# pixray/pixray

Measured on AMD Instinct MI355X. Metric: optimisation iters/sec, VQGAN 256^2 + ViT-B/32 + 64 cutouts, higher is better.
Workload: dtype fp16

## Files before the change

include/prx.h:

```cpp
#ifndef PRX_H_
#define PRX_H_
#include <stddef.h>
#include <stdint.h>

#ifdef __cplusplus
extern "C" {
#endif

#define PRX_ABI_VERSION 3

typedef void* prx_stream_t;

const char* prx_last_error(void);
int prx_abi_version(void);
int prx_device_info(int* cu_count, char* arch_name, int arch_name_len);


#define PRX_ACT_NONE 0
#define PRX_ACT_QUICKGELU 1
#define PRX_ACT_MUL_DQUICKGELU 2
#define PRX_ACT_RELU 3
#define PRX_ACT_MUL_RELUMASK 4
#define PRX_ACT_RELUMASK_POST 5
#define PRX_ACT_GELU 6
// ... 54 lines not shown
                           void* dST, int lddst, int rows, int cols, prx_stream_t s);
int prx_k_upsample2x_bwd(const float* hi, float* low, int NB, int Hl, int Wl, int C, prx_stream_t s);
int prx_k_nchw_to_nhwc(const float* in, float* out_f32, void* out_bf16, int NB, int C, int HW, int Cpad,
                       prx_stream_t s);
int prx_k_nhwc_to_nchw(const float* in, int ldc, float* out, int NB, int C, int HW, prx_stream_t s);
int prx_k_image_head_fwd(const float* x, int ldc, float* img, int NB, int C, int HW, prx_stream_t s);
int prx_k_image_head_bwd(const float* x, int ldc, const float* gimg, float* dx, void* dx_bf16, int ldo, int NB, int C,
                         int HW, prx_stream_t s);
int prx_k_mha_fwd(const void* qkv, void* out, int N, int T, int C, int heads, prx_stream_t s);
int prx_k_mha_bwd(const void* qkv, const void* dout, void* dqkv, int N, int T, int C, int heads, prx_stream_t s);

int prx_k_groupnorm_fwd_op(const void* x, const float* gamma, const float* beta, double* stats, void* out16, float* out_f32,
                           int NB, int P, int C, int swish, float eps, int zero_stats, int stats_ready, int h16, int s16,
                           prx_stream_t s);
int prx_k_groupnorm_bwd_op(const void* g, const void* x, const float* gamma, const float* beta, const double* fstats,
                           double* bstats, const void* add, float* dx, void* dx16, int NB, int P, int C, int swish, float eps,
                           int zero_stats, int stats_ready, int h16, int s16, prx_stream_t s);
int prx_k_layernorm_fwd_op(const void* x, long long ldx, const float* gamma, const float* beta, void* out16, float* out_f32,
                           float* mean, float* rstd, int rows, int C, float eps, int h16, int s16, prx_stream_t s);
int prx_k_layernorm_bwd_op(const void* g, long long ldg, const void* x, long long ldx, const float* gamma, const float* mean,
                           const float* rstd, const void* add, long long ldadd, float* dx, long long lddx, void* dx16,
                           long long lddxb, int rows, int C, int h16, int add_every, int s16, prx_stream_t s);
int prx_k_mha_fwd_op(const void* qkv, void* out, int N, int T, int C, int heads, int h16, prx_stream_t s);
int prx_k_mha_bwd_op(const void* qkv, const void* dout, void* dqkv, int N, int T, int C, int heads, int h16, prx_stream_t s);
int prx_k_mha_fwd_gen_op(const void* qkv, void* out, float* lse, int N, int T, int C, int heads, int h16, prx_stream_t s);
int prx_k_mha_bwd_gen_op(const void* qkv, const void* out, const void* dout, const float* lse, void* dqkv, int N, int T, int C,
                         int heads, int h16, prx_stream_t s);
int prx_k_mha_fwd_causal_op(const void* qkv, void* out, int N, int T, int C, int heads, int h16, prx_stream_t s);
int prx_k_softmax_rows_op(const float* S, int lds_, float scale, void* P, int ldp, void* PT, int ldpt, int rows, int cols,
                          int prec, prx_stream_t s);
int prx_k_softmax_rows_bwd_op(const void* P, int ldp, const float* dP, int lddp, float scale, void* dS, int ldds, void* dST,
                              int lddst, int rows, int cols, int prec, prx_stream_t s);
int prx_k_transpose_op(const void* in, int ldin, void* out, int ldout, int R, int C, int f32, prx_stream_t s);
int prx_k_upsample2x_bwd_op(const void* hi, float* low, void* low16, int NB, int Hl, int Wl, int C, int h16, int s16,
                            prx_stream_t s);
int prx_k_nchw_to_nhwc_op(const float* in, float* out_f32, void* out16, int NB, int C, int HW, int Cpad, int h16, prx_stream_t s);
int prx_k_image_head_bwd_op(const float* x, int ldc, const float* gimg, float* dx, void* dx16, int ldo, int NB, int C, int HW,
                            int h16, const float* gscale, prx_stream_t s);
int prx_k_image_head_bwd_im2col(const float* x, int ldc, const float* gimg, void* col, int ldk, int C, int H, int W, int h16,
                                const float* gscale, prx_stream_t s);
int prx_k_grad_scale(const float* g, size_t n, float* part, int nparts, int target_log2, float* scale2, prx_stream_t s);
int prx_k_grad_scale_multi(const float* const* gs, const size_t* ns, int count, float* part, int nparts_each, int target_log2,
                           float* scale2, prx_stream_t s);
int prx_k_scale_dev(float* x, size_t n, const float* scale, void* out16, int h16, prx_stream_t s);
int prx_k_f32_to_op16(const float* in, void* out16, size_t n, int h16, prx_stream_t s);
int prx_k_add_f32(const float* a, const float* b, float* out, size_t n, prx_stream_t s);

int prx_k_rn_pack_conv3x3(const float* w, void* Wf, void* Wd, int Cout, int Cin, int prec, prx_stream_t s);
int prx_k_stem1_fwd(const float* cut, const float* mm, const float* w, const float* b, void* out, int N, int S, int CO, int prec,
                    prx_stream_t s);
int prx_k_stem1_bwd(const void* g, const float* w, float* dY, int N, int S, int CO, const float* oscale_dev, int prec, prx_stream_t s);
int prx_k_avgpool2_fwd(const void* x, void* out, int N, int H, int W, int C, int prec, prx_stream_t s);
int prx_k_avgpool2_bwd(const float* g, const void* mask, float* dx_f32, void* dx_op, int N, int H, int W, int C, int prec,
                       prx_stream_t s);
int prx_k_relu_mask(float* g, const void* out, void* g_op, size_t n, int prec, prx_stream_t s);
int prx_k_tokens_fwd(const float* x, const float* pos, void* t, int N, int P, int C, int prec, prx_stream_t s);
int prx_k_tokens_bwd(const float* dt, float* dx, int N, int P, int C, int prec, prx_stream_t s);
int prx_k_tok0_gather(const void* t, void* out, int N, int T, int C, int prec, prx_stream_t s);
int prx_k_tok0_scatter(const void* g0, void* dt, int N, int T, int C, int prec, prx_stream_t s);
int prx_k_minmax(const float* x, size_t n, float* part, int nparts, float* mm, prx_stream_t s);
int prx_k_patchify_fwd(const float* cut, const float* mm, void* A, int prec, int N, int S, int P, int T, float m0, float m1, float m2,
                       float s0, float s1, float s2, prx_stream_t s);
int prx_k_patchify_bwd_reduce(const float* cut, const float* mm, const float* dA, double* acc, int N, int S, int P, int T, float m0,
                              float m1, float m2, float s0, float s1, float s2, prx_stream_t s);
int prx_k_patchify_bwd_apply(const float* cut, const float* mm, const float* dA, const double* acc, float* gcut, int N, int S, int P,
                             int T, float m0, float m1, float m2, float s0, float s1, float s2, prx_stream_t s);
// ... 285 lines not shown
```

pixray_amd/csrc/api_kernels.hip:

```cpp
#include "common.h"
#include "norms.h"
#include "elementwise.h"
#include "attention.h"
#include "resnet.h"
#include "cutouts.h"
#include "vgg.h"
#include "vit.h"
#include "clip_text.h"
#include "prompt_vq.h"
#include "vqgan.h"
#include "vqgan_enc.h"
#include "../../include/prx.h"

#define S_(x) ((hipStream_t)(x))
#define B_(x) ((bf16_t*)(x))
#define CB_(x) ((const bf16_t*)(x))

extern "C" {

int prx_k_groupnorm_fwd(const float* x, const float* gamma, const float* beta, double* stats, void* out_bf16,
                        float* out_f32, int NB, int P, int C, int swish, float eps, prx_stream_t s) {
    return prx_groupnorm_fwd(x, gamma, beta, stats, B_(out_bf16), out_f32, NB, P, C, swish, eps, S_(s));
}
int prx_k_groupnorm_bwd(const float* g, const float* x, const float* gamma, const float* beta, const double* fstats,
                        double* bstats, const float* add, float* dx, int NB, int P, int C, int swish, float eps,
                        prx_stream_t s) {
    return prx_groupnorm_bwd(g, x, gamma, beta, fstats, bstats, add, dx, nullptr, NB, P, C, swish, eps, S_(s));
}
int prx_k_layernorm_fwd(const float* x, long long ldx, const float* gamma, const float* beta, void* out_bf16,
                        float* out_f32, float* mean, float* rstd, int rows, int C, float eps, prx_stream_t s) {
    return prx_layernorm_fwd(x, ldx, gamma, beta, B_(out_bf16), out_f32, mean, rstd, rows, C, eps, S_(s));
}
int prx_k_layernorm_bwd(const float* g, long long ldg, const float* x, long long ldx, const float* gamma,
                        const float* mean, const float* rstd, const float* add, long long ldadd, float* dx,
                        long long lddx, int rows, int C, prx_stream_t s) {
    return prx_layernorm_bwd(g, ldg, x, ldx, gamma, mean, rstd, add, ldadd, dx, lddx, nullptr, 0, rows, C, S_(s));
}
int prx_k_transpose_bf16(const void* in, int ldin, void* out, int ldout, int R, int C, prx_stream_t s) {
    return prx_transpose_op(in, ldin, out, ldout, R, C, PRX_PREC_BF16, S_(s));
}
int prx_k_softmax_rows(const float* S, int lds_, float scale, void* P, int ldp, void* PT, int ldpt, int rows, int cols,
                       prx_stream_t s) {
    return prx_softmax_rows(S, lds_, scale, P, ldp, PT, ldpt, rows, cols, PRX_PREC_BF16, S_(s));
// ... 59 lines not shown
}
int prx_k_layernorm_bwd_op(const void* g, long long ldg, const void* x, long long ldx, const float* gamma, const float* mean,
                           const float* rstd, const void* add, long long ldadd, float* dx, long long lddx, void* dx16,
                           long long lddxb, int rows, int C, int h16, int add_every, int s16, prx_stream_t s) {
    return prx_layernorm_bwd(g, ldg, x, ldx, gamma, mean, rstd, add, ldadd, dx, lddx, B_(dx16), lddxb, rows, C, S_(s), h16,
                             add_every, s16);
}
int prx_k_mha_fwd_op(const void* qkv, void* out, int N, int T, int C, int heads, int h16, prx_stream_t s) {
    return prx_mha_fwd(CB_(qkv), B_(out), N, T, C, heads, S_(s), h16);
}
int prx_k_mha_bwd_op(const void* qkv, const void* dout, void* dqkv, int N, int T, int C, int heads, int h16, prx_stream_t s) {
    return prx_mha_bwd(CB_(qkv), CB_(dout), B_(dqkv), N, T, C, heads, S_(s), h16);
}
int prx_k_mha_fwd_gen_op(const void* qkv, void* out, float* lse, int N, int T, int C, int heads, int h16, prx_stream_t s) {
    return prx_mha_fwd_gen(CB_(qkv), B_(out), lse, N, T, C, heads, S_(s), h16);
}
int prx_k_mha_bwd_gen_op(const void* qkv, const void* out, const void* dout, const float* lse, void* dqkv, int N, int T, int C,
                         int heads, int h16, prx_stream_t s) {
    return prx_mha_bwd_gen(CB_(qkv), CB_(out), CB_(dout), lse, B_(dqkv), N, T, C, heads, S_(s), h16);
}
int prx_k_mha_fwd_causal_op(const void* qkv, void* out, int N, int T, int C, int heads, int h16, prx_stream_t s) {
    return prx_mha_fwd_causal(CB_(qkv), B_(out), N, T, C, heads, S_(s), h16);
}
int prx_k_softmax_rows_op(const float* S, int lds_, float scale, void* P, int ldp, void* PT, int ldpt, int rows, int cols,
                          int prec, prx_stream_t s) {
    PRX_REQUIRE(prec_valid(prec), "softmax_rows: unknown precision %d", prec);
    return prx_softmax_rows(S, lds_, scale, P, ldp, PT, ldpt, rows, cols, prec, S_(s));
}
int prx_k_softmax_rows_bwd_op(const void* P, int ldp, const float* dP, int lddp, float scale, void* dS, int ldds, void* dST,
                              int lddst, int rows, int cols, int prec, prx_stream_t s) {
    PRX_REQUIRE(prec_valid(prec), "softmax_rows_bwd: unknown precision %d", prec);
    return prx_softmax_rows_bwd(P, ldp, dP, lddp, scale, dS, ldds, dST, lddst, rows, cols, prec, S_(s));
}
int prx_k_transpose_op(const void* in, int ldin, void* out, int ldout, int R, int C, int f32, prx_stream_t s) {
    return prx_transpose_op(in, ldin, out, ldout, R, C, f32, S_(s));
}
int prx_k_upsample2x_bwd_op(const void* hi, float* low, void* low16, int NB, int Hl, int Wl, int C, int h16, int s16,
                            prx_stream_t s) {
    return prx_upsample2x_bwd(hi, low, B_(low16), NB, Hl, Wl, C, S_(s), h16, s16);
}
int prx_k_nchw_to_nhwc_op(const float* in, float* out_f32, void* out16, int NB, int C, int HW, int Cpad, int h16, prx_stream_t s) {
    return prx_nchw_to_nhwc(in, out_f32, B_(out16), NB, C, HW, Cpad, S_(s), h16);
}
int prx_k_image_head_bwd_op(const float* x, int ldc, const float* gimg, float* dx, void* dx16, int ldo, int NB, int C, int HW,
                            int h16, const float* gscale, prx_stream_t s) {
    return prx_image_head_bwd(x, ldc, gimg, dx, B_(dx16), ldo, NB, C, HW, S_(s), h16, gscale);
}
int prx_k_image_head_bwd_im2col(const float* x, int ldc, const float* gimg, void* col, int ldk, int C, int H, int W, int h16,
                                const float* gscale, prx_stream_t s) {
    return prx_image_head_bwd_im2col(x, ldc, gimg, B_(col), ldk, C, H, W, S_(s), h16, gscale);
}
int prx_k_grad_scale(const float* g, size_t n, float* part, int nparts, int target_log2, float* scale2, prx_stream_t s) {
    return prx_grad_scale(g, n, part, nparts, target_log2, scale2, S_(s));
}
int prx_k_grad_scale_multi(const float* const* gs, const size_t* ns, int count, float* part, int nparts_each, int target_log2,
                           float* scale2, prx_stream_t s) {
    return prx_grad_scale_multi(gs, ns, count, part, nparts_each, target_log2, scale2, S_(s));
}
int prx_k_scale_dev(float* x, size_t n, const float* scale, void* out16, int h16, prx_stream_t s) {
    return prx_scale_dev(x, n, scale, S_(s), B_(out16), h16);
}
int prx_k_f32_to_op16(const float* in, void* out16, size_t n, int h16, prx_stream_t s) {
    return prx_f32_to_bf16(in, B_(out16), n, S_(s), h16);
}
int prx_k_add_f32(const float* a, const float* b, float* out, size_t n, prx_stream_t s) {
    return prx_add_f32(a, b, out, n, S_(s));
// ... 104 lines not shown
```

pixray_amd/csrc/vqgan.hip:

```cpp
#include "vqgan.h"
#include "gemm.h"
#include "norms.h"
#include "elementwise.h"
#include "prompt_vq.h"
#include "vit.h"
#include <vector>
#include <memory>
#include <stdlib.h>

namespace {

template <typename TOp>
__global__ __launch_bounds__(256) void pack_conv3x3_kernel(const float* __restrict__ w, TOp* __restrict__ Wf,
                                                           TOp* __restrict__ Wd, int Cout, int Cin, int CoP) {
    const size_t total_f = (size_t)Cout * 9 * Cin;
    const size_t total_d = (size_t)Cin * 9 * CoP;
    for (size_t i = (size_t)blockIdx.x * blockDim.x + threadIdx.x; i < total_f + total_d;
         i += (size_t)gridDim.x * blockDim.x) {
        if (i < total_f) {
            int ci = (int)(i % Cin);
            int tap = (int)((i / Cin) % 9);
            int co = (int)(i / ((size_t)9 * Cin));
            Wf[i] = op_cvt<TOp>(w[(((size_t)co * Cin + ci) * 3 + tap / 3) * 3 + tap % 3]);
        } else {
            size_t j = i - total_f;
            int co = (int)(j % CoP);
            int tap = (int)((j / CoP) % 9);
            int ci = (int)(j / ((size_t)9 * CoP));
            int ky = 2 - tap / 3, kx = 2 - tap % 3;
            Wd[j] = op_cvt<TOp>((co < Cout) ? w[(((size_t)co * Cin + ci) * 3 + ky) * 3 + kx] : 0.f);
        }
    }
}

__global__ __launch_bounds__(256) void colminmax_kernel(const float* __restrict__ w, float* __restrict__ mn,
                                                        float* __restrict__ mx, int rows, int D) {
// ... 6 lines not shown

}

int prx_vqgan_pack_conv3x3(const float* w, void* Wf, void* Wd, int Cout, int Cin, int CoP, int prec, hipStream_t s) {
    PRX_REQUIRE(prec_valid(prec), "vqgan pack_conv3x3: unknown precision %d", prec);
    PRX_OP_DISPATCH(prec_is_f32(prec), prec_is_h16(prec), TO,
                    hipLaunchKernelGGL(pack_conv3x3_kernel<TO>, dim3(1024), dim3(256), 0, s, w, (TO*)Wf, (TO*)Wd, Cout, Cin, CoP));
    PRX_LAUNCH_CHECK();
    return 0;
}
int prx_colminmax(const float* w, float* mn, float* mx, int rows, int D, hipStream_t s) {
    hipLaunchKernelGGL(colminmax_kernel, dim3(ceil_div(D, 256)), dim3(256), 0, s, w, mn, mx, rows, D);
    PRX_LAUNCH_CHECK();
    return 0;
}

static inline int pad8(int P) { return (P + 7) & ~7; }

struct Conv3 { int Cin, Cout, CoP; void *Wf, *Wd; float* b; };
struct Conv1 { int Cin, Cout; void *W, *WT; float* b; };
struct GN { int C; float *g, *b; double *stats, *bstats; int id; };

struct ResBlock {
    int Cin, Cout, rh, rw;
    GN n1, n2; Conv3 c1, c2; Conv1 sc; bool has_sc;
    void *x_in, *h1, *scbuf, *out;
    void *x_in_bf, *out_bf;
};
struct AttnBlock {
    int C, rh, rw;
    GN n; Conv1 qkv, proj;
    void* x_in; void *qkvb, *Pm, *PT; void* out; void* out_bf;
    void* qkvT;
};
struct UpBlock { int C, rh, rw; Conv3 c; void *x_in, *out; void *x_in_bf, *out_bf; };

struct Stage { int kind; int idx; };

struct PrxVqgan {
    int zc, D, NC, ch, out_ch, h0, w0, H, W, nstage;
    int prec;
    int f32, h16;
    int lean;
    float* gs;
    GemmCtx gctx;
    std::vector<void*> allocs;
    float *codebook, *cnorm, *zmin, *zmax;
    Conv1 pq; Conv3 conv_in, conv_out; GN norm_out;
    std::vector<ResBlock> res; std::vector<AttnBlock> attn; std::vector<UpBlock> ups; std::vector<Stage> stages;
    float *zq, *y, *dzq; void* h_in; int* idx; void *pqo_bf, *h_in_bf, *dpq_bf;
    float *pmin; int* pidx;
    void* a;
    void *tA, *tB, *tC, *tD, *dqkv, *dy8;
    void *dycol, *Wd_col;
    float* S;
    void *g0, *g1, *g2;
    void *g0b, *g1b, *g2b;
    double* all_stats; int n_gn;
    float* ws; size_t ws_bytes;
    void* x_last;
};

namespace {
template <typename Tp>
int dalloc(PrxVqgan* v, Tp** p, size_t count) {
    void* q = nullptr;
    PRX_CHECK_HIP(hipMalloc(&q, std::max<size_t>(count, 1) * sizeof(Tp)));
    v->allocs.push_back(q);
    *p = (Tp*)q;
    return 0;
}
#define VALLOC(ptr, count) do { int _r = dalloc(v, &(ptr), (count)); if (_r) return _r; } while (0)
int dalloc_op(PrxVqgan* v, void** p, size_t count) {
    void* q = nullptr;
    PRX_CHECK_HIP(hipMalloc(&q, std::max<size_t>(count, 1) * op_esz(v->f32)));
    v->allocs.push_back(q);
// ... 58 lines not shown
    if ((r = make_gn(v, rb.n2, Cout, cur, s))) return r;
    if ((r = make_conv3(v, rb.c2, Cout, Cout, cur, s))) return r;
    const size_t P = (size_t)rh * rw;
    if (rb.has_sc) {
        if ((r = make_conv1(v, rb.sc, Cin, Cout, cur, s))) return r;
        VALLOC_S(rb.scbuf, P * Cout);
    }
    VALLOC_S(rb.h1, P * Cout); VALLOC_S(rb.out, P * Cout);
    v->stages.push_back({0, (int)v->res.size()});
    v->res.push_back(rb);
    return 0;
}
int make_attn(PrxVqgan* v, int C, int rh, int rw, WCursor& cur, hipStream_t s) {
    AttnBlock ab{};
    ab.C = C; ab.rh = rh; ab.rw = rw;
    int r;
    if ((r = make_gn(v, ab.n, C, cur, s))) return r;
    const float *wq, *bq, *wk, *bk, *wv, *bv;
    NEXTW(cur, wq); NEXTW(cur, bq); NEXTW(cur, wk); NEXTW(cur, bk); NEXTW(cur, wv); NEXTW(cur, bv);
    float *wcat, *bcat;
    VALLOC(wcat, (size_t)3 * C * C); VALLOC(bcat, 3 * C);
    const float* ws_[3] = {wq, wk, wv}; const float* bs_[3] = {bq, bk, bv};
    for (int i = 0; i < 3; ++i) {
        PRX_CHECK_HIP(hipMemcpyAsync(wcat + (size_t)i * C * C, ws_[i], sizeof(float) * C * C, hipMemcpyDeviceToDevice, s));
        PRX_CHECK_HIP(hipMemcpyAsync(bcat + i * C, bs_[i], sizeof(float) * C, hipMemcpyDeviceToDevice, s));
    }
    ab.qkv.Cin = C; ab.qkv.Cout = 3 * C; ab.qkv.b = bcat;
    VALLOC_OP(ab.qkv.W, (size_t)3 * C * C); VALLOC_OP(ab.qkv.WT, (size_t)3 * C * C);
    if ((r = prx_pack_op(wcat, ab.qkv.W, (size_t)3 * C * C, v->prec, s))) return r;
    if ((r = prx_pack_transpose_op(wcat, ab.qkv.WT, 3 * C, C, v->prec, s))) return r;
    if ((r = make_conv1(v, ab.proj, C, C, cur, s))) return r;
    const size_t P = (size_t)rh * rw;
    const size_t P8 = (size_t)pad8((int)P);
    VALLOC_OP(ab.qkvb, P * 3 * C); VALLOC_OP(ab.Pm, P * P8); VALLOC_OP(ab.PT, P * P8); VALLOC_S(ab.out, P * C);
    VALLOC_OP(ab.qkvT, (size_t)3 * C * P8);
    PRX_CHECK_HIP(hipMemsetAsync(ab.qkvT, 0, (size_t)3 * C * P8 * op_esz(v->f32), s));
    PRX_CHECK_HIP(hipMemsetAsync(ab.Pm, 0, P * P8 * op_esz(v->f32), s));
    PRX_CHECK_HIP(hipMemsetAsync(ab.PT, 0, P * P8 * op_esz(v->f32), s));
    v->stages.push_back({1, (int)v->attn.size()});
    v->attn.push_back(ab);
    return 0;
}
int make_up(PrxVqgan* v, int C, int rh, int rw, WCursor& cur, hipStream_t s) {
    UpBlock ub{};
    ub.C = C; ub.rh = rh; ub.rw = rw;
    int r;
    if ((r = make_conv3(v, ub.c, C, C, cur, s))) return r;
    VALLOC_S(ub.out, (size_t)rh * rw * C);
    v->stages.push_back({2, (int)v->ups.size()});
    v->ups.push_back(ub);
    return 0;
}
}

int prx_vqgan_create_impl(PrxVqgan** out, int ch, const int* ch_mult, int n_mult, int num_res_blocks, int attn_res,
                          int resolution, int z_channels, int embed_dim, int n_embed, int out_ch, int h0, int w0,
                          int precision, const float* const* w, int n_w, hipStream_t s) {
    PRX_REQUIRE(h0 >= 1 && w0 >= 1, "vqgan_create: bad latent size %dx%d", h0, w0);
    PRX_REQUIRE(prec_valid(precision), "vqgan_create: unknown precision %d", precision);
    PRX_REQUIRE(embed_dim == z_channels, "vqgan_create: embed_dim must equal z_channels");
    PrxVqgan* v = new PrxVqgan();
    std::unique_ptr<PrxVqgan> guard(v);
    v->prec = precision; v->f32 = prec_is_f32(precision); v->h16 = prec_is_h16(precision);
    v->gs = nullptr;
    { const char* e = getenv("PRX_LEAN"); v->lean = (v->h16 && !(e && atoi(e) == 0)) ? 1 : 0; }
    v->n_gn = 0; v->zc = z_channels; v->D = embed_dim; v->NC = n_embed; v->ch = ch; v->out_ch = out_ch; v->h0 = h0; v->w0 = w0;
    WCursor cur{w, n_w, 0};
    int r;
    const float* cb; NEXTW(cur, cb);
    if ((r = copyf(v, &v->codebook, cb, (size_t)n_embed * embed_dim, s))) return r;
    VALLOC(v->cnorm, n_embed); VALLOC(v->zmin, embed_dim); VALLOC(v->zmax, embed_dim);
    if ((r = prx_sqnorm_rows(v->codebook, v->cnorm, n_embed, embed_dim, s))) return r;
    if ((r = prx_colminmax(v->codebook, v->zmin, v->zmax, n_embed, embed_dim, s))) return r;
    if ((r = make_conv1(v, v->pq, embed_dim, z_channels, cur, s))) return r;
    int block_in = ch * ch_mult[n_mult - 1];
    int rh = h0, rw = w0;
    if ((r = make_conv3(v, v->conv_in, z_channels, block_in, cur, s))) return r;
    if ((r = make_res(v, block_in, block_in, rh, rw, cur, s))) return r;
    if ((r = make_attn(v, block_in, rh, rw, cur, s))) return r;
    if ((r = make_res(v, block_in, block_in, rh, rw, cur, s))) return r;
    int nominal = resolution >> (n_mult - 1);
    for (int lvl = n_mult - 1; lvl >= 0; --lvl) {
        int block_out = ch * ch_mult[lvl];
        for (int b = 0; b < num_res_blocks + 1; ++b) {
            if ((r = make_res(v, block_in, block_out, rh, rw, cur, s))) return r;
            block_in = block_out;
            if (nominal == attn_res) { if ((r = make_attn(v, block_in, rh, rw, cur, s))) return r; }
        }
        if (lvl != 0) {
            rh *= 2; rw *= 2; nominal *= 2;
            if ((r = make_up(v, block_in, rh, rw, cur, s))) return r;
        }
    }
    v->H = rh; v->W = rw;
    if ((r = make_gn(v, v->norm_out, block_in, cur, s))) return r;
    if ((r = make_conv3(v, v->conv_out, block_in, out_ch, cur, s))) return r;
    PRX_REQUIRE(cur.pos == n_w, "vqgan_create: %d weight tensors given, %d consumed", n_w, cur.pos);
    const size_t P0 = (size_t)h0 * w0, PH = (size_t)rh * rw;
// ... 168 lines not shown
    bool sr = nx && nx->C == v->conv_in.Cout && fusable(v, nx->C);
    void* x = v->h_in;
    void* x_bf = v->h_in_bf;
    for (int si = 0; si < (int)v->stages.size(); ++si) {
        const Stage& st = v->stages[si];
        nx = first_norm(v, si + 1);
        if (st.kind == 0) {
            ResBlock& b = v->res[st.idx];
            const int P = b.rh * b.rw;
            b.x_in = x; b.x_in_bf = x_bf;
            if ((r = gn_fwd(v, b.n1, x, P, 1, s, sr))) return r;
            if ((r = conv3_fwd(v, b.c1, v->a, false, b.rh, b.rw, false, nullptr, b.h1, b.Cout, s, nullptr, &b.n2))) return r;
            const void* resid = x;
            if (b.has_sc) {
                PRX_REQUIRE(x_bf != nullptr, "vqgan: missing bf16 twin for the shortcut input");
                GemmDesc d; d.A = x_bf; d.lda = b.Cin; d.B = b.sc.W; d.ldb = b.Cin; d.M = P; d.N = b.Cout; d.K = b.Cin;
                d.bias_n = b.sc.b; out_stream(v, d, b.scbuf, b.Cout, nullptr);
                if ((r = vg(v, d, s))) return r;
                resid = b.scbuf;
            }
            if ((r = gn_fwd(v, b.n2, b.h1, P, 1, s, fusable(v, b.Cout)))) return r;
            if ((r = conv3_fwd(v, b.c2, v->a, false, b.rh, b.rw, false, resid, b.out, b.Cout, s, b.out_bf, nx))) return r;
            sr = nx && nx->C == b.Cout && fusable(v, b.Cout);
            x = b.out; x_bf = b.out_bf;
        } else if (st.kind == 1) {
            AttnBlock& b = v->attn[st.idx];
            const int P = b.rh * b.rw, C = b.C;
            b.x_in = x;
            if ((r = gn_fwd(v, b.n, x, P, 0, s, sr))) return r;
            {   GemmDesc d; d.A = v->a; d.lda = C; d.B = b.qkv.W; d.ldb = C; d.M = P; d.N = 3 * C; d.K = C;
                d.bias_n = b.qkv.b; d.out_bf16 = b.qkvb; d.ldc_bf16 = 3 * C;
                if ((r = vg(v, d, s))) return r; }
            const int P8 = pad8(P);
            if ((r = prx_transpose_op(b.qkvb, 3 * C, b.qkvT, P8, P, 3 * C, v->f32, s))) return r;
            {   GemmDesc d; d.A = b.qkvb; d.lda = 3 * C; d.B = op_off(b.qkvb, C, v->f32); d.ldb = 3 * C; d.M = P; d.N = P; d.K = C;
                d.out_f32 = v->S; d.ldc_f32 = P;
                if ((r = vg(v, d, s))) return r; }
            if ((r = prx_softmax_rows(v->S, P, 1.f / sqrtf((float)C), b.Pm, P8, b.PT, P8, P, P, v->prec, s))) return r;
            {   GemmDesc d; d.A = b.Pm; d.lda = P8; d.B = op_off(b.qkvT, (size_t)2 * C * P8, v->f32); d.ldb = P8; d.M = P; d.N = C; d.K = P8;
                d.out_bf16 = v->tB; d.ldc_bf16 = C;
                if ((r = vg(v, d, s))) return r; }
            {   GemmDesc d; d.A = v->tB; d.lda = C; d.B = b.proj.W; d.ldb = C; d.M = P; d.N = C; d.K = C;
                d.bias_n = b.proj.b; resid_stream(v, d, x, C); out_stream(v, d, b.out, C, b.out_bf);
                if (nx && nx->C == C && fusable(v, C)) { d.gn_stats = nx->stats; d.gn_gs = C / 32; }
                if ((r = vg(v, d, s))) return r; }
            sr = nx && nx->C == C && fusable(v, C);
            x = b.out; x_bf = b.out_bf;
        } else {
            UpBlock& b = v->ups[st.idx];
            b.x_in = x; b.x_in_bf = x_bf;
            PRX_REQUIRE(x_bf != nullptr, "vqgan: missing bf16 twin for the upsample input");
            if ((r = conv3_fwd(v, b.c, x_bf, false, b.rh, b.rw, true, nullptr, b.out, b.C, s, b.out_bf, nx))) return r;
            sr = nx && nx->C == b.C && fusable(v, b.C);
            x = b.out; x_bf = b.out_bf;
        }
        {   const int Pq = st.kind == 0 ? v->res[st.idx].rh * v->res[st.idx].rw : st.kind == 1 ? v->attn[st.idx].rh * v->attn[st.idx].rw : v->ups[st.idx].rh * v->ups[st.idx].rw;
            const int Cq = st.kind == 0 ? v->res[st.idx].Cout : st.kind == 1 ? v->attn[st.idx].C : v->ups[st.idx].C;
            vq_trace(v, "fwd", si, x, (size_t)Pq * Cq, s); }
    }
    v->x_last = x;
    const int PH = v->H * v->W;
    if ((r = gn_fwd(v, v->norm_out, x, PH, 1, s, sr))) return r;
    if ((r = conv3_fwd(v, v->conv_out, v->a, false, v->H, v->W, false, nullptr, v->y, v->conv_out.CoP, s, nullptr, nullptr, true))) return r;
    return prx_image_head_fwd(v->y, v->conv_out.CoP, img, 1, v->out_ch, PH, s);
}

long long prx_vqgan_debug_stage_impl(PrxVqgan* v, int stage, float* dst, long long max_floats, hipStream_t s) {
    const void* src = nullptr; long long n = 0;
    PRX_REQUIRE(!v->lean || stage == -2 || stage >= (int)v->stages.size(), "vqgan debug_stage: the stage outputs are 16-bit in the lean layout (PRX_LEAN=0 for fp32 streams)");
    const int ns = (int)v->stages.size();
    if (stage == -2) { src = v->zq; n = (long long)v->h0 * v->w0 * v->D; }
    else if (stage == -1) { src = v->h_in; n = (long long)v->h0 * v->w0 * v->conv_in.Cout; }
    else if (stage >= 0 && stage < ns) {
        const Stage& st = v->stages[stage];
// ... 22 lines not shown
        out_stream(v, d, t1.f, v->conv_out.Cin, nullptr);
        set_gnb(v, d, &v->norm_out, v->x_last, 1);
        if ((r = vg(v, d, s))) return r;
    } else {
        if ((r = prx_image_head_bwd(v->y, v->conv_out.CoP, g_img, v->f32 ? (float*)v->dy8 : nullptr, v->f32 ? nullptr : (bf16_t*)v->dy8, v->conv_out.CoP, 1,
                                    v->out_ch, PH, s, v->h16, v->gs))) return r;
        if ((r = conv3_bwd(v, v->conv_out, v->dy8, false, v->H, v->W, t1.f, s, nullptr, &v->norm_out, v->x_last, 1))) return r;
    }
    if ((r = gn_bwd(v, v->norm_out, t1.f, v->x_last, nullptr, g.f, g.b, PH, 1, s, true))) return r;
    for (int si = (int)v->stages.size() - 1; si >= 0; --si) {
        const Stage& st = v->stages[si];
        if (st.kind == 0) {
            ResBlock& b = v->res[st.idx];
            const int P = b.rh * b.rw;
            if ((r = conv3_bwd(v, b.c2, g.b, false, b.rh, b.rw, t1.f, s, nullptr, &b.n2, b.h1, 1))) return r;
            if ((r = gn_bwd(v, b.n2, t1.f, b.h1, nullptr, v->f32 ? t2.f : nullptr, t2.b, P, 1, s, true))) return r;
            if ((r = conv3_bwd(v, b.c1, t2.b, false, b.rh, b.rw, t1.f, s, nullptr, &b.n1, b.x_in, 1))) return r;
            const void* add = g.f;
            if (b.has_sc) {
                GemmDesc d; d.A = g.b; d.lda = b.Cout; d.B = b.sc.WT; d.ldb = b.Cout; d.M = P; d.N = b.Cin; d.K = b.Cout;
                out_stream(v, d, t2.f, b.Cin, nullptr);
                if ((r = vg(v, d, s))) return r;
                add = t2.f;
            }
            GB& dst = (add == g.f) ? t2 : g;
            if ((r = gn_bwd(v, b.n1, t1.f, b.x_in, add, dst.f, dst.b, P, 1, s, true))) return r;
            if (&dst != &g) std::swap(g, t2);
        } else if (st.kind == 1) {
            AttnBlock& b = v->attn[st.idx];
            const int P = b.rh * b.rw, C = b.C;
            {   GemmDesc d; d.A = g.b; d.lda = C; d.B = b.proj.WT; d.ldb = C; d.M = P; d.N = C; d.K = C;
                d.out_bf16 = v->tA; d.ldc_bf16 = C;
                if ((r = vg(v, d, s))) return r; }
            {   GemmDesc d; d.A = v->tA; d.lda = C; d.B = op_off(b.qkvb, 2 * C, v->f32); d.ldb = 3 * C; d.M = P; d.N = P; d.K = C;
                d.out_f32 = v->S; d.ldc_f32 = P;
                if ((r = vg(v, d, s))) return r; }
            const int P8 = pad8(P);
            if ((r = zero_if_padded(v, v->tB, P, P, s))) return r;
            if ((r = zero_if_padded(v, v->tC, P, P, s))) return r;
            if ((r = prx_softmax_rows_bwd(b.Pm, P8, v->S, P, 1.f / sqrtf((float)C), v->tB, P8, v->tC, P8, P, P, v->prec, s))) return r;
            {   GemmDesc d; d.A = v->tB; d.lda = P8; d.B = op_off(b.qkvT, (size_t)C * P8, v->f32); d.ldb = P8; d.M = P; d.N = C; d.K = P8;
                d.out_bf16 = v->dqkv; d.ldc_bf16 = 3 * C;
                if ((r = vg(v, d, s))) return r; }
            {   GemmDesc d; d.A = v->tC; d.lda = P8; d.B = b.qkvT; d.ldb = P8; d.M = P; d.N = C; d.K = P8;
                d.out_bf16 = op_off(v->dqkv, C, v->f32); d.ldc_bf16 = 3 * C;
                if ((r = vg(v, d, s))) return r; }
            if ((r = zero_if_padded(v, v->tD, C, P, s))) return r;
            if ((r = prx_transpose_op(v->tA, C, v->tD, P8, P, C, v->f32, s))) return r;
            {   GemmDesc d; d.A = b.PT; d.lda = P8; d.B = v->tD; d.ldb = P8; d.M = P; d.N = C; d.K = P8;
                d.out_bf16 = op_off(v->dqkv, 2 * C, v->f32); d.ldc_bf16 = 3 * C;
                if ((r = vg(v, d, s))) return r; }
            {   GemmDesc d; d.A = v->dqkv; d.lda = 3 * C; d.B = b.qkv.WT; d.ldb = 3 * C; d.M = P; d.N = C; d.K = 3 * C;
                out_stream(v, d, t1.f, C, nullptr);
                set_gnb(v, d, &b.n, b.x_in, 0);
                if ((r = vg(v, d, s))) return r; }
            if ((r = gn_bwd(v, b.n, t1.f, b.x_in, g.f, t2.f, t2.b, P, 0, s, true))) return r;
            std::swap(g, t2);
        } else {
            UpBlock& b = v->ups[st.idx];
            if ((r = conv3_bwd(v, b.c, g.b, false, b.rh, b.rw, t1.f, s))) return r;
            if ((r = prx_upsample2x_bwd(t1.f, v->lean ? nullptr : (float*)t2.f, v->f32 ? nullptr : (bf16_t*)t2.b, 1, b.rh / 2, b.rw / 2, b.C, s, v->h16,
                                        v->lean))) return r;
            std::swap(g, t2);
        }
        {   const int Pq = st.kind == 0 ? v->res[st.idx].rh * v->res[st.idx].rw : st.kind == 1 ? v->attn[st.idx].rh * v->attn[st.idx].rw : v->ups[st.idx].rh * v->ups[st.idx].rw / 4;
            const int Cq = st.kind == 0 ? v->res[st.idx].Cin : st.kind == 1 ? v->attn[st.idx].C : v->ups[st.idx].C;
            vq_trace(v, "bwd", si, g.f, (size_t)Pq * Cq, s); }
    }
    if ((r = conv3_bwd(v, v->conv_in, g.b, false, v->h0, v->w0, v->lean ? nullptr : t1.f, s, v->dpq_bf))) return r;
    const int P0 = v->h0 * v->w0;
    {   GemmDesc d; d.A = v->dpq_bf; d.lda = v->zc; d.B = v->pq.WT; d.ldb = v->zc; d.M = P0; d.N = v->D; d.K = v->zc;
        d.out_f32 = v->dzq; d.ldc_f32 = v->D;
        if (v->h16) d.alpha_dev = v->gs + 1;
        if ((r = vg(v, d, s))) return r; }
    return prx_nhwc_to_nchw(v->dzq, v->D, dz, 1, v->D, P0, s);
}
```

Before: 161.7.

## Fuse VQGAN single-head attention into dedicated forward and backward MFMA kernels

Replaces the VQGAN decoder attention path (transpose, QK^T GEMM, softmax, PV GEMM, and the matching backward chain) with custom kernels that keep the score row in shared memory and compute softmax and the output product in one launch. Backward uses a row kernel for dS/dq plus a column kernel for dk/dv. The goal is to cut launches, the fp32 score round-trip through global memory, and the transposed buffers. In exchange it recomputes QK^T per column tile, is limited to P<=512 and 16-bit precisions, and adds new hand-written MFMA code whose correctness and occupancy are unproven.

```diff
diff --git a/include/prx.h b/include/prx.h
--- a/include/prx.h
+++ b/include/prx.h
@@ -110,6 +110,8 @@
 int prx_k_softmax_rows_bwd_op(const void* P, int ldp, const float* dP, int lddp, float scale, void* dS, int ldds, void* dST,
                               int lddst, int rows, int cols, int prec, prx_stream_t s);
 int prx_k_transpose_op(const void* in, int ldin, void* out, int ldout, int R, int C, int f32, prx_stream_t s);
+int prx_attn1h_fwd(const void* qkv, void* o, void* Pm, int P, int C, int prec, prx_stream_t s);
+int prx_attn1h_bwd(const void* qkv, const void* Pm, const void* dout, void* dS, void* dqkv, int P, int C, int prec, prx_stream_t s);
 int prx_k_upsample2x_bwd_op(const void* hi, float* low, void* low16, int NB, int Hl, int Wl, int C, int h16, int s16,
                             prx_stream_t s);
 int prx_k_nchw_to_nhwc_op(const float* in, float* out_f32, void* out16, int NB, int C, int HW, int Cpad, int h16, prx_stream_t s);
diff --git a/pixray_amd/csrc/api_kernels.hip b/pixray_amd/csrc/api_kernels.hip
--- a/pixray_amd/csrc/api_kernels.hip
+++ b/pixray_amd/csrc/api_kernels.hip
@@ -9,6 +9,7 @@
 #include "clip_text.h"
 #include "prompt_vq.h"
 #include "vqgan.h"
+#include "vqgan_attn.h"
 #include "vqgan_enc.h"
 #include "../../include/prx.h"
 
@@ -134,6 +135,12 @@
     PRX_REQUIRE(prec_valid(prec), "softmax_rows_bwd: unknown precision %d", prec);
     return prx_softmax_rows_bwd(P, ldp, dP, lddp, scale, dS, ldds, dST, lddst, rows, cols, prec, S_(s));
 }
+int prx_attn1h_fwd(const void* qkv, void* o, void* Pm, int P, int C, int prec, prx_stream_t s) {
+    return prx_attn1h_fwd_impl(qkv, o, Pm, P, C, prec, S_(s));
+}
+int prx_attn1h_bwd(const void* qkv, const void* Pm, const void* dout, void* dS, void* dqkv, int P, int C, int prec, prx_stream_t s) {
+    return prx_attn1h_bwd_impl(qkv, Pm, dout, dS, dqkv, P, C, prec, S_(s));
+}
 int prx_k_transpose_op(const void* in, int ldin, void* out, int ldout, int R, int C, int f32, prx_stream_t s) {
     return prx_transpose_op(in, ldin, out, ldout, R, C, f32, S_(s));
 }
diff --git a/pixray_amd/csrc/vqgan.hip b/pixray_amd/csrc/vqgan.hip
--- a/pixray_amd/csrc/vqgan.hip
+++ b/pixray_amd/csrc/vqgan.hip
@@ -2,6 +2,7 @@
 #include "gemm.h"
 #include "norms.h"
 #include "elementwise.h"
+#include "vqgan_attn.h"
 #include "prompt_vq.h"
 #include "vit.h"
 #include <vector>
@@ -74,6 +75,7 @@
     GN n; Conv1 qkv, proj;
     void* x_in; void *qkvb, *Pm, *PT; void* out; void* out_bf;
     void* qkvT;
+    bool fused;
 };
 struct UpBlock { int C, rh, rw; Conv3 c; void *x_in, *out; void *x_in_bf, *out_bf; };
 
@@ -84,6 +86,7 @@
     int prec;
     int f32, h16;
     int lean;
+    int attn_fused;
     float* gs;
     GemmCtx gctx;
     std::vector<void*> allocs;
@@ -208,11 +211,14 @@
     if ((r = make_conv1(v, ab.proj, C, C, cur, s))) return r;
     const size_t P = (size_t)rh * rw;
     const size_t P8 = (size_t)pad8((int)P);
-    VALLOC_OP(ab.qkvb, P * 3 * C); VALLOC_OP(ab.Pm, P * P8); VALLOC_OP(ab.PT, P * P8); VALLOC_S(ab.out, P * C);
-    VALLOC_OP(ab.qkvT, (size_t)3 * C * P8);
-    PRX_CHECK_HIP(hipMemsetAsync(ab.qkvT, 0, (size_t)3 * C * P8 * op_esz(v->f32), s));
+    ab.fused = v->attn_fused && prx_attn1h_takes((int)P, C);
+    VALLOC_OP(ab.qkvb, P * 3 * C); VALLOC_OP(ab.Pm, P * P8); VALLOC_S(ab.out, P * C);
     PRX_CHECK_HIP(hipMemsetAsync(ab.Pm, 0, P * P8 * op_esz(v->f32), s));
-    PRX_CHECK_HIP(hipMemsetAsync(ab.PT, 0, P * P8 * op_esz(v->f32), s));
+    if (!ab.fused) {
+        VALLOC_OP(ab.PT, P * P8); VALLOC_OP(ab.qkvT, (size_t)3 * C * P8);
+        PRX_CHECK_HIP(hipMemsetAsync(ab.qkvT, 0, (size_t)3 * C * P8 * op_esz(v->f32), s));
+        PRX_CHECK_HIP(hipMemsetAsync(ab.PT, 0, P * P8 * op_esz(v->f32), s));
+    }
     v->stages.push_back({1, (int)v->attn.size()});
     v->attn.push_back(ab);
     return 0;
@@ -240,6 +246,7 @@
     v->prec = precision; v->f32 = prec_is_f32(precision); v->h16 = prec_is_h16(precision);
     v->gs = nullptr;
     { const char* e = getenv("PRX_LEAN"); v->lean = (v->h16 && !(e && atoi(e) == 0)) ? 1 : 0; }
+    { const char* e = getenv("PRX_VQ_ATTN_FUSED"); v->attn_fused = (!v->f32 && !(e && atoi(e) == 0)) ? 1 : 0; }
     v->n_gn = 0; v->zc = z_channels; v->D = embed_dim; v->NC = n_embed; v->ch = ch; v->out_ch = out_ch; v->h0 = h0; v->w0 = w0;
     WCursor cur{w, n_w, 0};
     int r;
@@ -474,6 +481,9 @@
                 d.bias_n = b.qkv.b; d.out_bf16 = b.qkvb; d.ldc_bf16 = 3 * C;
                 if ((r = vg(v, d, s))) return r; }
             const int P8 = pad8(P);
+            if (b.fused) {
+                if ((r = prx_attn1h_fwd_impl(b.qkvb, v->tB, b.Pm, P, C, v->prec, s))) return r;
+            } else {
             if ((r = prx_transpose_op(b.qkvb, 3 * C, b.qkvT, P8, P, 3 * C, v->f32, s))) return r;
             {   GemmDesc d; d.A = b.qkvb; d.lda = 3 * C; d.B = op_off(b.qkvb, C, v->f32); d.ldb = 3 * C; d.M = P; d.N = P; d.K = C;
                 d.out_f32 = v->S; d.ldc_f32 = P;
@@ -482,6 +492,7 @@
             {   GemmDesc d; d.A = b.Pm; d.lda = P8; d.B = op_off(b.qkvT, (size_t)2 * C * P8, v->f32); d.ldb = P8; d.M = P; d.N = C; d.K = P8;
                 d.out_bf16 = v->tB; d.ldc_bf16 = C;
                 if ((r = vg(v, d, s))) return r; }
+            }
             {   GemmDesc d; d.A = v->tB; d.lda = C; d.B = b.proj.W; d.ldb = C; d.M = P; d.N = C; d.K = C;
                 d.bias_n = b.proj.b; resid_stream(v, d, x, C); out_stream(v, d, b.out, C, b.out_bf);
                 if (nx && nx->C == C && fusable(v, C)) { d.gn_stats = nx->stats; d.gn_gs = C / 32; }
@@ -570,6 +581,9 @@
             {   GemmDesc d; d.A = g.b; d.lda = C; d.B = b.proj.WT; d.ldb = C; d.M = P; d.N = C; d.K = C;
                 d.out_bf16 = v->tA; d.ldc_bf16 = C;
                 if ((r = vg(v, d, s))) return r; }
+            if (b.fused) {
+                if ((r = prx_attn1h_bwd_impl(b.qkvb, b.Pm, v->tA, v->tB, v->dqkv, P, C, v->prec, s))) return r;
+            } else {
             {   GemmDesc d; d.A = v->tA; d.lda = C; d.B = op_off(b.qkvb, 2 * C, v->f32); d.ldb = 3 * C; d.M = P; d.N = P; d.K = C;
                 d.out_f32 = v->S; d.ldc_f32 = P;
                 if ((r = vg(v, d, s))) return r; }
@@ -588,6 +602,7 @@
             {   GemmDesc d; d.A = b.PT; d.lda = P8; d.B = v->tD; d.ldb = P8; d.M = P; d.N = C; d.K = P8;
                 d.out_bf16 = op_off(v->dqkv, 2 * C, v->f32); d.ldc_bf16 = 3 * C;
                 if ((r = vg(v, d, s))) return r; }
+            }
             {   GemmDesc d; d.A = v->dqkv; d.lda = 3 * C; d.B = b.qkv.WT; d.ldb = 3 * C; d.M = P; d.N = C; d.K = 3 * C;
                 out_stream(v, d, t1.f, C, nullptr);
                 set_gnb(v, d, &b.n, b.x_in, 0);
diff --git a/pixray_amd/csrc/vqgan_attn.h b/pixray_amd/csrc/vqgan_attn.h
--- /dev/null
+++ b/pixray_amd/csrc/vqgan_attn.h
@@ -0,0 +1,6 @@
+#pragma once
+#include "common.h"
+#define PRX_ATTN1H_PMAX 512
+static inline bool prx_attn1h_takes(int P, int C) { return P >= 1 && P <= PRX_ATTN1H_PMAX && C >= 64 && C % 64 == 0; }
+int prx_attn1h_fwd_impl(const void* qkv, void* o, void* Pm, int P, int C, int prec, hipStream_t s);
+int prx_attn1h_bwd_impl(const void* qkv, const void* Pm, const void* dout, void* dS, void* dqkv, int P, int C, int prec, hipStream_t s);
diff --git a/pixray_amd/csrc/vqgan_attn.hip b/pixray_amd/csrc/vqgan_attn.hip
--- /dev/null
+++ b/pixray_amd/csrc/vqgan_attn.hip
@@ -0,0 +1,311 @@
+#include "vqgan_attn.h"
+#include <math.h>
+
+namespace {
+
+typedef __attribute__((ext_vector_type(2))) _Float16 f16x2_t;
+
+template <typename T> struct A16;
+template <> struct A16<half_t> {
+    using x8 = f16x8; using x4 = f16x4; using x2 = f16x2_t;
+    static __device__ __forceinline__ f32x4 mma(x8 a, x8 b, f32x4 c) { return __builtin_amdgcn_mfma_f32_16x16x32_f16(a, b, c, 0, 0, 0); }
+};
+template <> struct A16<bf16_t> {
+    using x8 = bf16x8; using x4 = bf16x4; using x2 = bf16x2;
+    static __device__ __forceinline__ f32x4 mma(x8 a, x8 b, f32x4 c) { return __builtin_amdgcn_mfma_f32_16x16x32_bf16(a, b, c, 0, 0, 0); }
+};
+
+constexpr int QT = 16;
+constexpr int NC = 128;
+constexpr int KC = 64;
+constexpr int ZP = NC + 4;
+constexpr int YP = QT + 4;
+constexpr int PMAX = PRX_ATTN1H_PMAX;
+constexpr int SP = PMAX + 4;
+constexpr int PP = PMAX + 8;
+constexpr int ZBUF = 2 * KC * ZP;
+constexpr int SZ_FLOATS = (QT * SP > ZBUF / 2) ? QT * SP : ZBUF / 2;
+
+template <typename T>
+__device__ __forceinline__ void chunk_get(const T* __restrict__ Z, int ld, int k0, int n0, int P, int C, int tid,
+                                          typename A16<T>::x8 (&v)[4]) {
+    using V8 = typename A16<T>::x8;
+#pragma unroll
+    for (int i = 0; i < 4; ++i) {
+        const int piece = tid + 256 * i;
+        const int gr = k0 + (piece >> 4), col = n0 + 8 * (piece & 15);
+        const bool ok = gr < P && col < C;
+        const V8 x = *reinterpret_cast<const V8*>(Z + (size_t)(ok ? gr : 0) * ld + (ok ? col : 0));
+        const V8 z = {0, 0, 0, 0, 0, 0, 0, 0};
+        v[i] = ok ? x : z;
+    }
+}
+template <typename T>
+__device__ __forceinline__ void chunk_put(const typename A16<T>::x8 (&v)[4], T* Zs, int tid) {
+    using V4 = typename A16<T>::x4;
+#pragma unroll
+    for (int i = 0; i < 4; ++i) {
+        const int piece = tid + 256 * i;
+        T* d = Zs + (piece >> 4) * ZP + 8 * (piece & 15);
+        *reinterpret_cast<V4*>(d) = __builtin_shufflevector(v[i], v[i], 0, 1, 2, 3);
+        *reinterpret_cast<V4*>(d + 4) = __builtin_shufflevector(v[i], v[i], 4, 5, 6, 7);
+    }
+}
+
+template <typename T, bool TRA>
+__device__ __forceinline__ void chunk_mma(const T* As, const T* Zs, int wave, int lane, f32x4& acc_e, f32x4& acc_o) {
+    using V8 = typename A16<T>::x8;
+    using V2 = typename A16<T>::x2;
+    const int r = lane & 15, g = lane >> 4;
+#pragma unroll
+    for (int t = 0; t < KC / 32; ++t) {
+        V8 a, be, bo;
+        if constexpr (TRA) {
+#pragma unroll
+            for (int s = 0; s < 8; ++s) a[s] = As[(32 * t + 8 * g + s) * YP + r];
+        } else {
+            a = *reinterpret_cast<const V8*>(As + r * PP + 32 * t + 8 * g);
+        }
+#pragma unroll
+        for (int s = 0; s < 8; ++s) {
+            const V2 d = *reinterpret_cast<const V2*>(Zs + (32 * t + 8 * g + s) * ZP + 32 * wave + 2 * r);
+            be[s] = d[0];
+            bo[s] = d[1];
+        }
+        acc_e = A16<T>::mma(a, be, acc_e);
+        acc_o = A16<T>::mma(a, bo, acc_o);
+    }
+}
+
+template <typename T>
+__device__ __forceinline__ void store_pairs(const f32x4& acc_e, const f32x4& acc_o, T* __restrict__ out, int ldo, int m0, int M,
+                                            int n0, int C, int wave, int lane) {
+    using V2 = typename A16<T>::x2;
+    const int col = n0 + 32 * wave + 2 * (lane & 15);
+    if (col >= C) return;
+#pragma unroll
+    for (int i = 0; i < 4; ++i) {
+        const int row = m0 + 4 * (lane >> 4) + i;
+        if (row < M) {
+            V2 o;
+            o[0] = op_cvt<T>(acc_e[i]);
+            o[1] = op_cvt<T>(acc_o[i]);
+            *reinterpret_cast<V2*>(out + (size_t)row * ldo + col) = o;
+        }
+    }
+}
+
+template <typename T, bool BWD>
+__global__ __launch_bounds__(256) void attn1h_row_kernel(const T* __restrict__ X, int ldx, const T* __restrict__ Y,
+                                                         const T* __restrict__ Z, int ldyz, T* __restrict__ Pm, int ldp,
+                                                         T* __restrict__ dS, T* __restrict__ out, int ldo, int P, int C,
+                                                         float scale) {
+    using V8 = typename A16<T>::x8;
+    __shared__ __attribute__((aligned(16))) float Sz[SZ_FLOATS];
+    __shared__ __attribute__((aligned(16))) T Pl[QT * PP];
+    const int tid = threadIdx.x, wave = tid >> 6, lane = tid & 63;
+    const int r = lane & 15, g = lane >> 4;
+    const int q0 = blockIdx.x * QT, n0 = blockIdx.y * NC;
+    const int Pk = (P + KC - 1) & ~(KC - 1);
+
+    {
+        const int nkb = (P + 15) >> 4;
+        const T* xrow = X + (size_t)min(q0 + r, P - 1) * ldx;
+        for (int kb0 = 4 * wave; kb0 < nkb; kb0 += 16) {
+            const T* yrow[4];
+#pragma unroll
+            for (int u = 0; u < 4; ++u) yrow[u] = Y + (size_t)min(16 * (kb0 + u) + r, P - 1) * ldyz;
+            f32x4 acc[4];
+#pragma unroll
+            for (int u = 0; u < 4; ++u) acc[u] = f32x4{0.f, 0.f, 0.f, 0.f};
+            V8 an[2], bn[2][4];
+            auto request = [&](int c0) {
+#pragma unroll
+                for (int h = 0; h < 2; ++h) {
+                    const int c = c0 + 16 * g + 8 * h;
+                    an[h] = *reinterpret_cast<const V8*>(xrow + c);
+#pragma unroll
+                    for (int u = 0; u < 4; ++u) bn[h][u] = *reinterpret_cast<const V8*>(yrow[u] + c);
+                }
+            };
+            request(0);
+            for (int c0 = 0; c0 < C; c0 += 64) {
+                V8 a[2], b[2][4];
+#pragma unroll
+                for (int h = 0; h < 2; ++h) {
+                    a[h] = an[h];
+#pragma unroll
+                    for (int u = 0; u < 4; ++u) b[h][u] = bn[h][u];
+                }
+                request(min(c0 + 64, C - 64));
+#pragma unroll
+                for (int h = 0; h < 2; ++h)
+#pragma unroll
+                    for (int u = 0; u < 4; ++u) acc[u] = A16<T>::mma(a[h], b[h][u], acc[u]);
+            }
+#pragma unroll
+            for (int u = 0; u < 4; ++u)
+                if (kb0 + u < nkb) {
+#pragma unroll
+                    for (int i = 0; i < 4; ++i) Sz[(4 * g + i) * SP + 16 * (kb0 + u) + r] = acc[u][i];
+                }
+        }
+    }
+    __syncthreads();
+    V8 zr[4];
+    chunk_get<T>(Z, ldyz, 0, n0, P, C, tid, zr);
+
+    {
+        const bool wr = blockIdx.y == 0;
+        const float* s0 = Sz + (4 * wave) * SP;
+        T* p0 = Pl + (4 * wave) * PP;
+        if constexpr (!BWD) {
+            float mx[4], sum[4];
+#pragma unroll
+            for (int i = 0; i < 4; ++i) { mx[i] = -INFINITY; sum[i] = 0.f; }
+            for (int c = lane; c < P; c += 64)
+#pragma unroll
+                for (int i = 0; i < 4; ++i) mx[i] = fmaxf(mx[i], s0[i * SP + c] * scale);
+#pragma unroll
+            for (int i = 0; i < 4; ++i) mx[i] = wave_max(mx[i]);
+            for (int c = lane; c < P; c += 64)
+#pragma unroll
+                for (int i = 0; i < 4; ++i) sum[i] += __expf(s0[i * SP + c] * scale - mx[i]);
+#pragma unroll
+            for (int i = 0; i < 4; ++i) sum[i] = 1.f / wave_sum(sum[i]);
+            for (int c = lane; c < Pk; c += 64)
+#pragma unroll
+                for (int i = 0; i < 4; ++i) {
+                    const float sv = s0[i * SP + (c < P ? c : 0)];
+                    const T p = c < P ? op_cvt<T>(__expf(sv * scale - mx[i]) * sum[i]) : (T)0.f;
+                    p0[i * PP + c] = p;
+                    const int row = q0 + 4 * wave + i;
+                    if (wr && row < P && c < ldp) Pm[(size_t)row * ldp + c] = p;
+                }
+        } else {
+            float dot[4];
+#pragma unroll
+            for (int i = 0; i < 4; ++i) dot[i] = 0.f;
+            for (int c = lane; c < P; c += 64)
+#pragma unroll
+                for (int i = 0; i < 4; ++i) {
+                    const int row = min(q0 + 4 * wave + i, P - 1);
+                    dot[i] += (float)Pm[(size_t)row * ldp + c] * s0[i * SP + c];
+                }
+#pragma unroll
+            for (int i = 0; i < 4; ++i) dot[i] = wave_sum(dot[i]);
+            for (int c = lane; c < Pk; c += 64)
+#pragma unroll
+                for (int i = 0; i < 4; ++i) {
+                    const int row = q0 + 4 * wave + i, cc = c < P ? c : 0;
+                    const float p = (float)Pm[(size_t)min(row, P - 1) * ldp + cc];
+                    const T v = c < P ? op_cvt<T>(scale * p * (s0[i * SP + cc] - dot[i])) : (T)0.f;
+                    p0[i * PP + c] = v;
+                    if (wr && row < P && c < ldp) dS[(size_t)row * ldp + c] = v;
+                }
+        }
+    }
+    __syncthreads();
+
+    T* Zs = reinterpret_cast<T*>(Sz);
+    chunk_put<T>(zr, Zs, tid);
+    __syncthreads();
+    f32x4 acc_e = {0.f, 0.f, 0.f, 0.f}, acc_o = {0.f, 0.f, 0.f, 0.f};
+    const int nch = Pk / KC;
+    for (int ch = 0; ch < nch; ++ch) {
+        chunk_get<T>(Z, ldyz, KC * min(ch + 1, nch - 1), n0, P, C, tid, zr);
+        chunk_mma<T, false>(Pl + KC * ch, Zs + (ch & 1) * (KC * ZP), wave, lane, acc_e, acc_o);
+        chunk_put<T>(zr, Zs + ((ch + 1) & 1) * (KC * ZP), tid);
+        __syncthreads();
+    }
+    store_pairs<T>(acc_e, acc_o, out, ldo, q0, P, n0, C, wave, lane);
+}
+
+template <typename T>
+__global__ __launch_bounds__(256) void attn1h_col_kernel(const T* __restrict__ dS, const T* __restrict__ Pm, int ldp,
+                                                         const T* __restrict__ Q, int ldq, const T* __restrict__ dO, int lddo,
+                                                         T* __restrict__ dk, T* __restrict__ dv, int ldout, int P, int C) {
+    using V8 = typename A16<T>::x8;
+    using V4 = typename A16<T>::x4;
+    __shared__ __attribute__((aligned(16))) T Zs[ZBUF];
+    __shared__ __attribute__((aligned(16))) T Ys[2 * KC * YP];
+    const int tid = threadIdx.x, wave = tid >> 6, lane = tid & 63;
+    const int j0 = blockIdx.x * QT, n0 = blockIdx.y * NC;
+    const bool second = blockIdx.z != 0;
+    const T* __restrict__ Ysrc = second ? Pm : dS;
+    const T* __restrict__ Xsrc = second ? dO : Q;
+    const int ldx = second ? lddo : ldq;
+    T* __restrict__ out = second ? dv : dk;
+    const int nch = (P + KC - 1) / KC;
+    const int srow = (tid & 127) >> 1, scol = j0 + 8 * (tid & 1);
+
+    auto strip_get = [&](int i0) -> V8 {
+        const int gi = i0 + srow;
+        const bool ok = gi < P && scol < ldp;
+        const V8 x = *reinterpret_cast<const V8*>(Ysrc + (size_t)(ok ? gi : 0) * ldp + (ok ? scol : 0));
+        const V8 z = {0, 0, 0, 0, 0, 0, 0, 0};
+        return ok ? x : z;
+    };
+    auto strip_put = [&](const V8& v, T* dst) {
+        if (tid < 128) {
+            T* d = dst + srow * YP + 8 * (tid & 1);
+            *reinterpret_cast<V4*>(d) = __builtin_shufflevector(v, v, 0, 1, 2, 3);
+            *reinterpret_cast<V4*>(d + 4) = __builtin_shufflevector(v, v, 4, 5, 6, 7);
+        }
+    };
+
+    V8 zr[4];
+    chunk_get<T>(Xsrc, ldx, 0, n0, P, C, tid, zr);
+    V8 yr = strip_get(0);
+    chunk_put<T>(zr, Zs, tid);
+    strip_put(yr, Ys);
+    __syncthreads();
+    f32x4 acc_e = {0.f, 0.f, 0.f, 0.f}, acc_o = {0.f, 0.f, 0.f, 0.f};
+    for (int ch = 0; ch < nch; ++ch) {
+        const int nx = KC * min(ch + 1, nch - 1);
+        chunk_get<T>(Xsrc, ldx, nx, n0, P, C, tid, zr);
+        yr = strip_get(nx);
+        chunk_mma<T, true>(Ys + (ch & 1) * (KC * YP), Zs + (ch & 1) * (KC * ZP), wave, lane, acc_e, acc_o);
+        chunk_put<T>(zr, Zs + ((ch + 1) & 1) * (KC * ZP), tid);
+        strip_put(yr, Ys + ((ch + 1) & 1) * (KC * YP));
+        __syncthreads();
+    }
+    store_pairs<T>(acc_e, acc_o, out, ldout, j0, P, n0, C, wave, lane);
+}
+
+inline int pad8(int P) { return (P + 7) & ~7; }
+
+template <typename T>
+int fwd_t(const void* qkv, void* o, void* Pm, int P, int C, hipStream_t s) {
+    const T* q = (const T*)qkv;
+    hipLaunchKernelGGL((attn1h_row_kernel<T, false>), dim3((P + QT - 1) / QT, (C + NC - 1) / NC), dim3(256), 0, s, q, 3 * C, q + C,
+                       q + 2 * C, 3 * C, (T*)Pm, pad8(P), (T*)nullptr, (T*)o, C, P, C, 1.f / sqrtf((float)C));
+    PRX_LAUNCH_CHECK();
+    return 0;
+}
+template <typename T>
+int bwd_t(const void* qkv, const void* Pm, const void* dout, void* dS, void* dqkv, int P, int C, hipStream_t s) {
+    const T* q = (const T*)qkv;
+    T* dq = (T*)dqkv;
+    const dim3 grid((P + QT - 1) / QT, (C + NC - 1) / NC);
+    hipLaunchKernelGGL((attn1h_row_kernel<T, true>), grid, dim3(256), 0, s, (const T*)dout, C, q + 2 * C, q + C, 3 * C,
+                       const_cast<T*>((const T*)Pm), pad8(P), (T*)dS, dq, 3 * C, P, C, 1.f / sqrtf((float)C));
+    PRX_LAUNCH_CHECK();
+    hipLaunchKernelGGL((attn1h_col_kernel<T>), dim3(grid.x, grid.y, 2), dim3(256), 0, s, (const T*)dS, (const T*)Pm, pad8(P), q,
+                       3 * C, (const T*)dout, C, dq + C, dq + 2 * C, 3 * C, P, C);
+    PRX_LAUNCH_CHECK();
+    return 0;
+}
+
+}
+
+int prx_attn1h_fwd_impl(const void* qkv, void* o, void* Pm, int P, int C, int prec, hipStream_t s) {
+    PRX_REQUIRE(prec == PRX_PREC_BF16 || prec == PRX_PREC_F16, "attn1h_fwd: 16-bit operand precisions only (got %d)", prec);
+    PRX_REQUIRE(prx_attn1h_takes(P, C), "attn1h_fwd: needs 1 <= P <= %d and C a multiple of 64 (got P %d, C %d)", PRX_ATTN1H_PMAX, P, C);
+    return prec_is_h16(prec) ? fwd_t<half_t>(qkv, o, Pm, P, C, s) : fwd_t<bf16_t>(qkv, o, Pm, P, C, s);
+}
+int prx_attn1h_bwd_impl(const void* qkv, const void* Pm, const void* dout, void* dS, void* dqkv, int P, int C, int prec, hipStream_t s) {
+    PRX_REQUIRE(prec == PRX_PREC_BF16 || prec == PRX_PREC_F16, "attn1h_bwd: 16-bit operand precisions only (got %d)", prec);
+    PRX_REQUIRE(prx_attn1h_takes(P, C), "attn1h_bwd: needs 1 <= P <= %d and C a multiple of 64 (got P %d, C %d)", PRX_ATTN1H_PMAX, P, C);
+    return prec_is_h16(prec) ? bwd_t<half_t>(qkv, Pm, dout, dS, dqkv, P, C, s) : bwd_t<bf16_t>(qkv, Pm, dout, dS, dqkv, P, C, s);
+}
```

New measurement: 162.0, median of 6. No clear change (+0.2%).
